# qway/nerfmeshes

Measured on AMD Instinct MI355X. Metric: rendered rays/sec (64+128 samples, 8x256 MLP), lego scene geometry, higher is better.
Workload: dtype f32; 1 GPU; nerf-synthetic lego: 8x256 coarse+fine MLP, 64 coarse + 128 fine samples, 800x800 view per step per rank, bounds [2,6], seeded weights/orbit poses; chunk_rays=65536, parallelism=single GPU

## Files before the change

### nerfmeshes_amd/csrc/mlp_device_r3.h

```cpp
#pragma once
#include "mlp_device.h"

namespace nm {

struct NextChunks {
    const char* s0; int b0;
    const char* s1; int b1;
};

template <int NT, int KS1, int KS2, int NW, int LDSBUF, int KCH>
__device__ __forceinline__ void gemm_stage3(f32x4 (&acc)[NT], const float (&b1)[KS1],
                                            const float (&b2)[(KS2 > 0 ? KS2 : 1)], const char* gw,
                                            const NextChunks nx, char* lds, int& slot, f32x4 (&carry)[2],
                                            int wave, int lane) {
    constexpr int KS = KS1 + KS2;
    constexpr int NCH = (KS + KCH - 1) / KCH;
    constexpr int NB = NT / 4;
    constexpr int STEP_BYTES = NT * 256;
    static_assert(NT % 4 == 0 && NB >= 1, "tile count");
    static_assert(NCH >= 2, "every stage must span at least two chunks (DMA runs two chunks ahead)");
    f32x4 ab[3];
    ab[0] = carry[0];
    ab[1] = carry[1];
#pragma unroll
    for (int c = 0; c < NCH; ++c) {
        const int steps = (KS - c * KCH) < KCH ? (KS - c * KCH) : KCH;
        const int nblk = steps * NB;
        const int slot1 = slot == 2 ? 0 : slot + 1;
        const int slot2 = slot1 == 2 ? 0 : slot1 + 1;
        const char* src;
        int bytes;
        if (c + 2 < NCH) {
            const int nsteps = (KS - (c + 2) * KCH) < KCH ? (KS - (c + 2) * KCH) : KCH;
            src = gw + (c + 2) * KCH * STEP_BYTES; bytes = nsteps * STEP_BYTES;
        } else if (c + 2 == NCH) { src = nx.s0; bytes = nx.b0; }
        else { src = nx.s1; bytes = nx.b1; }
        char* dst = lds + slot2 * LDSBUF;
        const char* buf = lds + slot * LDSBUF + lane * 16;
        const char* nbuf = lds + slot1 * LDSBUF + lane * 16;
#pragma unroll
        for (int j = 0; j < nblk; ++j) {
            if (j == 0 && wave < NW / 2) stream_to_lds<NW>(src, dst, bytes, wave, lane);
            if (j == nblk / 2 && wave >= NW / 2) stream_to_lds<NW>(src, dst, bytes, wave, lane);
            const int ks = j / NB, blk = j % NB;
            const int s = c * KCH + ks;
            const float b = s < KS1 ? b1[s < KS1 ? s : 0] : b2[s >= KS1 ? s - KS1 : 0];
            const char* from = (j + 2 < nblk) ? buf + (j + 2) * 1024 : nbuf + (j + 2 - nblk) * 1024;
            const int r0 = (c * KCH * NB + j) % 3;
            ab[(r0 + 2) % 3] = *reinterpret_cast<const f32x4*>(from);
            __builtin_amdgcn_sched_barrier(0);
#pragma unroll
            for (int q = 0; q < 4; ++q)
                acc[blk * 4 + q] = __builtin_amdgcn_mfma_f32_16x16x4f32(ab[r0][q], b, acc[blk * 4 + q], 0, 0, 0);
        }
        __syncthreads();
        slot = slot1;
    }
    constexpr int TOTAL = KS * NB;
    carry[0] = ab[TOTAL % 3];
    carry[1] = ab[(TOTAL + 1) % 3];
}

template <int H, int FX, int FD, int NW, int KCH, bool FLAT = false, bool SKIP = false>
__global__ __launch_bounds__(NW * 64, H <= 128 ? 4 : 2) void mlp_kernel3(const MlpArgs args, const int num_layers,
                                                          const int density_only) {
    using N = Net<H, FX, FD, KCH>;
    static_assert(!(FLAT && SKIP), "the use_viewdirs = 0 heads have no colour branch to skip");
    static_assert(N::EX > KCH && N::KH >= 2 * KCH, "stages must span two chunks");
    extern __shared__ __attribute__((aligned(16))) char lds[];
    float* lds_bias = reinterpret_cast<float*>(lds + 3 * N::LDSBUF);
    const int nbias = H * (1 + num_layers) + H / 2 + 4;
    float* lds_walpha = lds_bias + nbias;
    float* lds_wrgb = lds_walpha + H;
    int* lds_vote = reinterpret_cast<int*>(lds_wrgb + 3 * H / 2);
    uint32_t* lds_claim = reinterpret_cast<uint32_t*>(lds_vote + 1);
    if (SKIP && threadIdx.x == 0) *lds_vote = 0;
    for (int i = threadIdx.x; i < nbias; i += NW * 64) lds_bias[i] = args.bias[i];
    for (int i = threadIdx.x; i < H; i += NW * 64) lds_walpha[i] = args.walpha[i];
    for (int i = threadIdx.x; i < ((FLAT && density_only == 2) ? 3 * H : 3 * H / 2); i += NW * 64) lds_wrgb[i] = args.wrgb[i];
    const int lane = threadIdx.x & 63;
    const int wave = __builtin_amdgcn_readfirstlane(threadIdx.x >> 6);
    const int g = lane >> 4, col = lane & 15;
    const float* tail_bias = lds_bias + nbias - 4;

    const int64_t wg_iters = mlp_wg_iters(args, NW * 16);
    auto hidden_next = [](const char* p) {
        return NextChunks{p, KCH * N::STEP, p + KCH * N::STEP, (N::KH - KCH < KCH ? N::KH - KCH : KCH) * N::STEP};
    };
    auto enc_next = [](const char* p, bool on) {
        return NextChunks{p, on ? KCH * N::STEP : 0, p + KCH * N::STEP,
                          on ? (N::EX - KCH < KCH ? N::EX - KCH : KCH) * N::STEP : 0};
    };
    auto dir_next = [](const char* p) { return NextChunks{p, KCH * N::STEPD, p + KCH * N::STEPD, KCH * N::STEPD}; };

    int slot = 0;
    f32x4 carry[2];
    if ((int64_t)blockIdx.x < wg_iters) {
        const NextChunks first = enc_next(args.wstream, true);
        stream_to_lds<NW>(first.s0, lds, first.b0, wave, lane);
        stream_to_lds<NW>(first.s1, lds + N::LDSBUF, first.b1, wave, lane);
    }
    __syncthreads();
    carry[0] = *reinterpret_cast<const f32x4*>(lds + lane * 16);
    carry[1] = *reinterpret_cast<const f32x4*>(lds + lane * 16 + 1024);

    int64_t next_it = 0;
    int turn = 0;
    constexpr bool TERM = SKIP && H > 128;
    const bool term = TERM && args.att != nullptr;
    auto att_entry = [&](int64_t t, uint32_t& k) -> float* {
        k = (uint32_t)t / args.att_blocks;
        return args.att + ((size_t)(uint32_t)t * NW + wave);
    };
    bool dead = false;
    auto claim_tile = [&](float& pre) -> uint32_t {
        uint32_t c = 0;
        if (lane == 0) c = atomicAdd(args.tile_queue, 1u);
        c = (uint32_t)__builtin_amdgcn_readfirstlane((int)c);
        pre = 0.0f;
        if (term) {
            const int64_t nx = (int64_t)gridDim.x + c;
            if (nx < wg_iters && nx >= (int64_t)args.att_blocks && lane < NW)
                pre = __hip_atomic_load(args.att + ((size_t)((uint32_t)nx - args.att_blocks) * NW + lane), __ATOMIC_RELAXED,
                                        __HIP_MEMORY_SCOPE_AGENT);
        }
        return c;
    };
    auto claim_word = [&](uint32_t c, float pre) -> uint32_t {
        const bool all_dead = term && __ballot(lane < NW && !(pre < -160.0f)) == 0;
        return c | (all_dead ? 0x80000000u : 0u);
    };
    for (int64_t it = blockIdx.x; it < wg_iters; it = SKIP ? next_it : it + gridDim.x) {
        bool has_next = !SKIP && it + gridDim.x < wg_iters;
        int64_t sample = (it * NW + wave) * 16 + col;
        bool valid = sample < args.n;
        if (SKIP && args.ray_tiles) {
            const uint32_t depth_slots = (uint32_t)args.samples >> 4;
            const uint32_t div = term ? args.att_blocks : depth_slots;
            const uint32_t q = (uint32_t)it / div, r = (uint32_t)it - q * div;
            const uint32_t block = term ? r : q;
            const int64_t ray_first = ((int64_t)block * NW + wave) * args.samples;
            sample = ray_first + ((term ? q : r) << 4) + col;
            valid = ray_first < args.n;
        }
        if (TERM && dead) {
            if (valid && g == 0) {
                f32x4 o4 = {0.0f, 0.0f, 0.0f, 0.0f};
                *reinterpret_cast<f32x4*>(args.out + 4 * sample) = o4;
            }
            uint32_t k;
            float* const entry = att_entry(it, k);
            if (lane == 0) __hip_atomic_store(entry, -1e30f, __ATOMIC_RELAXED, __HIP_MEMORY_SCOPE_AGENT);
            if (args.dead_count && threadIdx.x == 0) atomicAdd(args.dead_count, 1u);
            if (wave == 0) {
                float pre;
                const uint32_t c = claim_tile(pre);
                const uint32_t word = claim_word(c, pre);
                if (lane == 0) lds_claim[turn] = word;
            }
            __syncthreads();
            const uint32_t word = (uint32_t)__builtin_amdgcn_readfirstlane((int)lds_claim[turn]);
            turn ^= 1;
            next_it = (int64_t)gridDim.x + (word & 0x7fffffffu);
            dead = (word >> 31) != 0;
            continue;
        }
        const int64_t sidx = valid ? sample : args.n - 1;
        const SamplePD smp = fetch_sample(args, sidx);
        const float p[3] = {smp.px, smp.py, smp.pz}, d[3] = {smp.dx, smp.dy, smp.dz};
        const float dummy[1] = {0.0f};
        float encx[N::EX];
        encode<FX, N::EX>(encx, p, args.bands_xyz, g);
        NextChunks wrap = enc_next(args.wstream, has_next);

        f32x4 acc[N::NT];
        float in[N::KH];
        const char* gw = args.wstream;
        load_bias<N::NT>(acc, lds_bias, g);
        gemm_stage3<N::NT, N::EX, 0, NW, N::LDSBUF, KCH>(acc, encx, dummy, gw, hidden_next(gw + N::EX * N::STEP), lds, slot, carry, wave, lane);
        gw += N::EX * N::STEP;
        acc_to_operand<N::NT, false>(acc, in);
        if constexpr (TERM) {
            if (wave == 0) {
                float pre;
                const uint32_t claimed = claim_tile(pre);
                const uint32_t word = claim_word(claimed, pre);
                if (lane == 0) lds_claim[turn] = word;
            }
        } else if (SKIP && threadIdx.x == 0) lds_claim[turn] = atomicAdd(args.tile_queue, 1u);

        float sigma = 0.0f;
        bool empty_tile = false;
        const int trunk_iters = density_only ? num_layers - 1 : num_layers;
#pragma unroll 1
        for (int i = 0; i < trunk_iters; ++i) {
            const bool is_feat = i == num_layers - 1;
            float t_here = 0.0f, t_after = 0.0f, att_before = 0.0f;
            float* entry = nullptr;
            bool last_of_ray = false;
            if (term && is_feat) {
                uint32_t k;
                entry = att_entry(it, k);
                last_of_ray = (k << 4) + col + 1 == (uint32_t)args.samples;
                if (valid) {
                    t_here = args.c[sample];
                    if (!last_of_ray) t_after = args.c[sample + 1];
                    if (lane == 0 && k > 0)
                        att_before = __hip_atomic_load(entry - (size_t)args.att_blocks * NW, __ATOMIC_RELAXED, __HIP_MEMORY_SCOPE_AGENT);
                }
            }
            if (is_feat) sigma = alpha_gemv<H>(in, lds_walpha, g) + tail_bias[0];
            if (term && is_feat) {
                const float dist = (last_of_ray ? 1e10f : t_after - t_here) * nm_norm3(d[0], d[1], d[2]);
                const float a = 1.0f - expf(-(fmaxf(sigma, 0.0f) * dist));
                float c = log2f(((1.0f - a) + 1e-10f) + 0x1p-23f) + 0x1p-8f;
#pragma unroll
                for (int m = 1; m < 16; m <<= 1) c += __shfl_xor(c, m);
                if (lane == 0)
                    __hip_atomic_store(entry, valid ? att_before + c : -1e30f, __ATOMIC_RELAXED, __HIP_MEMORY_SCOPE_AGENT);
            }
            if (SKIP && is_feat) {
                const int epoch = (int)it + 1;
                const bool dense = valid && !(sigma <= 0.0f);
                if (dense) *lds_vote = epoch;
                __syncthreads();
                empty_tile = __builtin_amdgcn_readfirstlane(*lds_vote) != epoch;
                const uint32_t word = (uint32_t)__builtin_amdgcn_readfirstlane((int)lds_claim[turn]);
                next_it = (int64_t)gridDim.x + (word & 0x7fffffffu);
                dead = (word >> 31) != 0;
                turn ^= 1;
                has_next = next_it < wg_iters;
                wrap = enc_next(args.wstream, has_next);
                if (empty_tile) break;
            }
            const bool skip = !is_feat && ((args.skip_mask >> i) & 1u);
            const bool last_density = density_only && i == num_layers - 2;
            load_bias<N::NT>(acc, lds_bias + H * (1 + i), g);
            {
                const char* after = gw + N::KH * N::STEP;
                NextChunks nx = hidden_next(after);
                if (skip) nx = enc_next(after, true);
                else if (is_feat) nx = dir_next(after);
                else if (last_density) nx = wrap;
                gemm_stage3<N::NT, N::KH, 0, NW, N::LDSBUF, KCH>(acc, in, dummy, gw, nx, lds, slot, carry, wave, lane);
                gw = after;
            }
            if (skip) {
                const char* after = gw + N::EX * N::STEP;
                const NextChunks nx = last_density ? wrap : hidden_next(after);
                gemm_stage3<N::NT, N::EX, 0, NW, N::LDSBUF, KCH>(acc, encx, dummy, gw, nx, lds, slot, carry, wave, lane);
                gw = after;
            }
            acc_to_operand<N::NT, true>(acc, in);
        }

        if (empty_tile) {
            if (valid && g == 0) {
                f32x4 o4 = {0.0f, 0.0f, 0.0f, sigma};
                *reinterpret_cast<f32x4*>(args.out + 4 * sample) = o4;
            }
            if (args.skip_count && threadIdx.x == 0) atomicAdd(args.skip_count, 1u);
            if (has_next) {
                const int slot1 = slot == 2 ? 0 : slot + 1;
                const int slot2 = slot1 == 2 ? 0 : slot1 + 1;
                stream_to_lds<NW>(wrap.s0, lds + slot1 * N::LDSBUF, wrap.b0, wave, lane);
                stream_to_lds<NW>(wrap.s1, lds + slot2 * N::LDSBUF, wrap.b1, wave, lane);
                __syncthreads();
                slot = slot1;
                carry[0] = *reinterpret_cast<const f32x4*>(lds + slot * N::LDSBUF + lane * 16);
                carry[1] = *reinterpret_cast<const f32x4*>(lds + slot * N::LDSBUF + lane * 16 + 1024);
            }
            continue;
        }

        if (density_only) {
            sigma = alpha_gemv<H>(in, lds_walpha, g) + tail_bias[0];
            if (FLAT && density_only == 2) flat_head<H>(args, in, lds_wrgb, tail_bias, sigma, sample, valid, g);
            else if (valid && g == 0) args.out[sample] = sigma;
            continue;
        }

        f32x4 accd[N::NTD];
        float v[N::KD];
        load_bias<N::NTD>(accd, lds_bias + H * (1 + num_layers), g);
        float encd[N::ED];
        encode<FD, N::ED>(encd, d, args.bands_dir, g);
        gemm_stage3<N::NTD, N::KH, N::ED, NW, N::LDSBUF, KCH>(accd, in, encd, gw, wrap, lds, slot, carry, wave, lane);
        acc_to_operand<N::NTD, true>(accd, v);

        float rgb[3];
#pragma unroll
        for (int ch = 0; ch < 3; ++ch) {
            float part = 0.0f;
            const float* wr = lds_wrgb + (ch * 4 + g) * N::KD;
#pragma unroll
            for (int s = 0; s < N::KD; s += 4) {
                const f32x4 w4 = *reinterpret_cast<const f32x4*>(wr + s);
#pragma unroll
                for (int q = 0; q < 4; ++q) part = fmaf(v[s + q], w4[q], part);
            }
            const float x = group_sum(part) + tail_bias[1 + ch];
            rgb[ch] = 1.0f / (1.0f + expf(-x));
        }
        if (valid && g == 0) {
            f32x4 o4 = {rgb[0], rgb[1], rgb[2], sigma};
            *reinterpret_cast<f32x4*>(args.out + 4 * sample) = o4;
        }
    }
}

}
```

### nerfmeshes_amd/csrc/nerf_mlp.hip

```cpp
#include <cstdlib>
#include <iterator>
#include <vector>

#include "nm_internal.h"
#include "mlp_device.h"
#include "mlp_device_r3.h"
#include "mlp_device_b3.h"
#include "mlp_device_g.h"

namespace nm {

template <int H, int FX, int FD, int NW, int KCH>
static MlpPlan make_plan() {
    return MlpPlan{H, FX, FD, NW, KCH, 0, 2 * Net<H, FX, FD, KCH>::LDSBUF, &mlp_kernel<H, FX, FD, NW, KCH, false>,
                   NW * 16, 8 / NW, &mlp_kernel<H, FX, FD, NW, KCH, false, true>, 0, nullptr, nullptr};
}

template <int H, int FX, int FD, int NW, int KCH, bool SKIP = true>
static MlpPlan make_plan3() {
    return MlpPlan{H, FX, FD, NW, KCH, 0, 3 * Net<H, FX, FD, KCH>::LDSBUF, &mlp_kernel3<H, FX, FD, NW, KCH>,
                   NW * 16, 8 / NW, &mlp_kernel3<H, FX, FD, NW, KCH, true>, 0, nullptr, nullptr,
                   SKIP ? &mlp_kernel3<H, FX, FD, NW, KCH, false, SKIP> : nullptr};
}

static const MlpPlan g_tuned_plans[] = {
    make_plan3<256, 10, 4, 8, 8>(),
    make_plan3<128, 10, 4, 8, 8>(),
    make_plan<64, 10, 4, 8, 8>(),
    make_plan3<256, 6, 4, 8, 8>(),
    make_plan3<128, 6, 4, 8, 8, false>(),
    make_plan<64, 6, 4, 8, 8>(),
};

void generic_plans_a(std::vector<MlpPlan>&);
void generic_plans_b(std::vector<MlpPlan>&);
void generic_plans_c(std::vector<MlpPlan>&);
void generic_plans_d(std::vector<MlpPlan>&);
void generic_plans_s(std::vector<MlpPlan>&);
void generic_plans_a_long(std::vector<MlpPlan>&);
void generic_plans_b_long(std::vector<MlpPlan>&);
void generic_plans_c_long(std::vector<MlpPlan>&);
void generic_plans_d_long(std::vector<MlpPlan>&);
void generic_plans_s_long(std::vector<MlpPlan>&);
void generic_plans_s_long_upper(std::vector<MlpPlan>&);

static const std::vector<MlpPlan>& all_plans() {
    static const std::vector<MlpPlan> plans = [] {
        std::vector<MlpPlan> v(std::begin(g_tuned_plans), std::end(g_tuned_plans));
        generic_plans_a(v); generic_plans_b(v); generic_plans_c(v); generic_plans_d(v); generic_plans_s(v);
        generic_plans_a_long(v); generic_plans_b_long(v); generic_plans_c_long(v); generic_plans_d_long(v); generic_plans_s_long(v); generic_plans_s_long_upper(v);
        return v;
    }();
    return plans;
}

struct B3Plan {
    int H, FX, FD;
    void (*kernel)(const MlpArgs, const int, const int);
    int chunk_units;
};
static const B3Plan g_b3_plans[] = {
    {256, 10, 4, &mlp_kernel_b3<256, 10, 4, 8>, B3_CHUNK_UNITS},
    {256, 6, 4, &mlp_kernel_b3<256, 6, 4, 8>, B3_CHUNK_UNITS},
    {128, 10, 4, &mlp_kernel_b3<128, 10, 4, 8, 8>, 8},
    {128, 6, 4, &mlp_kernel_b3<128, 6, 4, 8, 8>, 8},
    {64, 10, 4, &mlp_kernel_b3<64, 10, 4, 8, 3>, 3},
    {64, 6, 4, &mlp_kernel_b3<64, 6, 4, 8, 3>, 3},
};
static const B3Plan* find_b3_plan(int H, int FX, int FD) {
    for (const B3Plan& p : g_b3_plans)
        if (p.H == H && p.FX == FX && p.FD == FD) return &p;
    return nullptr;
}
bool has_b3_kernel(int H, int FX, int FD) { return find_b3_plan(H, FX, FD) != nullptr; }

const MlpPlan* find_mlp_plan(int H, int FX, int FD) {
    for (const MlpPlan& p : all_plans())
        if (!p.generic_nt && p.H == H && p.FX == FX && p.FD == FD) return &p;
    return nullptr;
}

const MlpPlan* find_generic_plan(int H, int L, bool long_encoding) {
    const int want = long_encoding ? G_LONG_VARIANT : 0;
    for (const MlpPlan& p : all_plans())
        if (p.generic_nt && p.variant == want && p.H >= H && forward_lds_bytes(p, H, L, 0) <= 160 * 1024) return &p;
    return nullptr;
}

int mlp_plan_info(const MlpPlan* p, int* nw) {
    *nw = p->NW;
    return p->generic_nt ? 1000 + p->generic_nt : p->variant;
}

int forward_lds_bytes(const MlpPlan& p, int H, int L, int head_floats) {
    if (p.generic_nt)
        return g_lds_bytes(p.ring_bytes, p.generic_nt, L, p.variant == G_LONG_VARIANT ? G_ENC_PARTS : 1);
    return p.ring_bytes + tuned_cache_bytes(H, L, head_floats);
}

static bool ray_termination_enabled() {
    const char* e = std::getenv("NM_RAY_TERMINATION");
    return !(e && e[0] == '0' && e[1] == 0);
}

int launch_mlp(const nm_mlp* m, const MlpArgs& args_in, int density_only, hipStream_t stream) {
    const MlpPlan* p = m->plan;
    if (args_in.n <= 0) return 0;
    MlpArgs args = args_in;
    if (!(args.skip_empty && p->kernel_skip && density_only == 0 && m->precision == NM_PREC_F32)) args.skip_empty = 0;
    args.ray_tiles = args.skip_empty && (args.mode == MODE_RAYS || args.mode == MODE_VIEW) && args.samples % 16 == 0;
    if (args.ray_tiles && mlp_wg_iters(args, p->wg_samples) > INT32_MAX) args.ray_tiles = 0;
    if (args.skip_empty && (!m->d_tile_queue || mlp_wg_iters(args, p->wg_samples) > INT32_MAX)) args.skip_empty = args.ray_tiles = 0;
    args.tile_queue = nullptr;
    if (!args.skip_empty) args.skip_count = nullptr;
    float* const att = args.ray_tiles ? args.att : nullptr;
    args.att = nullptr;
    args.att_blocks = 0;
    DeviceGuard guard(m->device);
    const int L = m->desc.num_layers, H = m->desc.hidden_size;
    NM_REQUIRE(density_only != 2 || (m->precision == NM_PREC_F32 && p->kernel_flat), "no kernel for use_viewdirs=0 networks in this plan");
    auto kernel = density_only == 2 ? p->kernel_flat : (args.skip_empty ? p->kernel_skip : p->kernel);
    if (m->precision == NM_PREC_BF16X3) {
        const B3Plan* b = find_b3_plan(H, m->desc.num_encoding_fn_xyz, m->desc.num_encoding_fn_dir);
        NM_REQUIRE(b && m->d_stream_b3, "no bf16x3 kernel for this network");
        const int lds_bytes = 3 * b->chunk_units * B3_UNIT + tuned_cache_bytes(H, L, 3 * H / 2 + 32);
        NM_REQUIRE(lds_bytes <= 160 * 1024, "LDS budget exceeded (bf16x3 ring + bias cache): too many layers");
        if (int rc = ensure_dynamic_lds((const void*)b->kernel, lds_bytes)) return rc;
        MlpArgs a = args;
        a.wstream = static_cast<const char*>(m->d_stream_b3);
        const unsigned grid = persistent_grid((a.n + 127) / 128, m->num_cus);
        hipLaunchKernelGGL(b->kernel, dim3(grid), dim3(512), lds_bytes, stream, a, L, density_only);
        NM_HIP_CHECK(hipGetLastError());
        return 0;
    }
    const int lds_bytes = forward_lds_bytes(*p, H, L, density_only == 2 ? 3 * H : 3 * H / 2);
    NM_REQUIRE(lds_bytes <= 160 * 1024, "LDS budget exceeded (ring + bias cache)");
    if (int rc = ensure_dynamic_lds((const void*)kernel, lds_bytes)) return rc;
    const int64_t wg_iters = mlp_wg_iters(args, p->wg_samples);
    unsigned grid = persistent_grid(wg_iters, (int64_t)m->num_cus * p->wg_per_cu);
    if (args.skip_empty) {
        const int64_t resident = (int64_t)m->num_cus * p->wg_per_cu * (p->H <= 128 ? 2 : 1);
        grid = (unsigned)(wg_iters < resident ? wg_iters : resident);
        args.tile_queue = m->d_tile_queue + (size_t)(__atomic_fetch_add(&m->tile_queue_turn, 1u, __ATOMIC_RELAXED) % TILE_QUEUE_SLOTS) * TILE_QUEUE_STRIDE;
        NM_HIP_CHECK(hipMemsetAsync(args.tile_queue, 0, sizeof(uint32_t), stream));
        const int64_t depth_slots = args.samples / 16, ray_blocks = att ? wg_iters / depth_slots : 0;
        const int64_t table = depth_slots * ray_blocks * p->NW;
        if (att && p->H > 128 && ray_blocks >= 2 * (int64_t)grid && table <= args.att_floats && ray_termination_enabled()) {
            args.att = att;
            args.att_blocks = (uint32_t)ray_blocks;
            NM_HIP_CHECK(hipMemsetAsync(att, 0, (size_t)table * sizeof(float), stream));
        }
    }
    if (!args.att) args.dead_count = nullptr;
    hipLaunchKernelGGL(kernel, dim3(grid), dim3(p->NW * 64), lds_bytes, stream, args, (int)m->desc.num_layers, density_only);
    NM_HIP_CHECK(hipGetLastError());
    return 0;
}

}
```

### nerfmeshes_amd/csrc/nm_internal.h

```cpp
#pragma once
#include <hip/hip_runtime.h>
#include <stdint.h>
#include <stdio.h>
#include <string.h>
#include <string>

#include "../../include/nerfmeshes_hip.h"
#include "mlp_pack.h"

namespace nm {

void set_error(const std::string& msg);

#define NM_HIP_CHECK(expr)                                                                   \
    do {                                                                                     \
        hipError_t _e = (expr);                                                              \
        if (_e != hipSuccess) {                                                              \
            ::nm::set_error(std::string(#expr) + ": " + hipGetErrorString(_e));              \
            return 1;                                                                        \
        }                                                                                    \
    } while (0)

#define NM_REQUIRE(cond, msg)                                                                \
    do {                                                                                     \
        if (!(cond)) {                                                                       \
            ::nm::set_error(std::string(msg) + " [" #cond "]");                              \
            return 2;                                                                        \
        }                                                                                    \
    } while (0)

constexpr int KC = 8;
constexpr int MAX_FREQ_XYZ = 32;
constexpr int MAX_FREQ_DIR = 32;

enum MlpMode : int { MODE_POINTS = 0, MODE_RAYS = 1, MODE_GRID = 2, MODE_VIEW = 3 };

struct RayGen {
    float rot[9];
    float origin[3];
    int32_t height, width;
    float focal;
    int32_t enabled;
    int32_t ndc;
    float ndc_near, c_w, c_h, two_near, m_two_near;
    int64_t first;
};

__device__ __forceinline__ float nm_norm3(float x, float y, float z) {
    return sqrtf(fmaf(z, z, fmaf(y, y, x * x)));
}

__device__ __forceinline__ void nm_ndc_ray(float near32, float c_w, float c_h, float two_near, float m_two_near,
                                           float (&o)[3], float (&d)[3]) {
    const float t = -(near32 + o[2]) / d[2];
    float q[3];
#pragma unroll
    for (int a = 0; a < 3; ++a) { const float td = t * d[a]; q[a] = o[a] + td; }
    const float o0 = (c_w * q[0]) / q[2];
    const float o1 = (c_h * q[1]) / q[2];
    const float rq = 1.0f / q[2];
    const float o2 = 1.0f + rq * two_near;
    const float d0 = c_w * (d[0] / d[2] - q[0] / q[2]);
    const float d1 = c_h * (d[1] / d[2] - q[1] / q[2]);
    const float d2 = rq * m_two_near;
    o[0] = o0; o[1] = o1; o[2] = o2;
    d[0] = d0; d[1] = d1; d[2] = d2;
}

__device__ __forceinline__ void nm_gen_ray(const RayGen& g, int64_t ray, float (&o)[3], float (&d)[3]) {
    const int64_t pix = g.first + ray;
    const int row = (int)(pix / g.width), colx = (int)(pix - (int64_t)row * g.width);
    const float x = ((float)colx - (float)(g.width * 0.5)) / g.focal;
    const float y = -((float)row - (float)(g.height * 0.5)) / g.focal;
    const float z = -1.0f;
    const float n = nm_norm3(x, y, z);
    const float dx = x / n, dy = y / n, dz = z / n;
#pragma unroll
    for (int a = 0; a < 3; ++a) {
        d[a] = (dx * g.rot[3 * a] + dy * g.rot[3 * a + 1]) + dz * g.rot[3 * a + 2];
        o[a] = g.origin[a];
    }
    if (g.ndc) nm_ndc_ray(g.ndc_near, g.c_w, g.c_h, g.two_near, g.m_two_near, o, d);
}

struct MlpArgs {
    const char* wstream;
    const float* bias;
    const float* walpha;
    const float* wrgb;
    float bands_xyz[MAX_FREQ_XYZ];
    float bands_dir[MAX_FREQ_DIR];
    uint32_t skip_mask;
    int32_t mode;
    const float* a;
    const float* b;
    const float* c;
    int64_t n;
    int64_t first;
    int32_t samples;
    int32_t origins_per_ray;
    int32_t n1, n2;
    float* out;
    float* tape_h;
    float* tape_feat;
    float* tape_v;
    uint64_t* mask_h;
    uint64_t* mask_v;
    int64_t tiles;
    float* tape_encx;
    float* tape_encd;
    int32_t tape_v_ld;
    int32_t tape_skip_h0;
    RayGen gen;
    const void* g_tab;
    int32_t g_nsx, g_idx, g_chx;
    int32_t g_nsd, g_idd, g_chd;
    int32_t g_h, g_hd;
    int32_t skip_empty;
    int32_t ray_tiles;
    uint32_t* skip_count;
    uint32_t* tile_queue;
    float* att;
    int64_t att_floats;
    uint32_t att_blocks;
    uint32_t* dead_count;
};

__host__ __device__ inline int64_t mlp_wg_iters(const MlpArgs& a, int wg_samples) {
    if (a.ray_tiles) {
        const int rays_per_tile = wg_samples / 16;
        return (a.n / a.samples + rays_per_tile - 1) / rays_per_tile * (a.samples / 16);
    }
    return (a.n + wg_samples - 1) / wg_samples;
}

struct MlpBwdArgs {
    const char* wstream;
    const float* walpha;
    const float* wrgb;
    const float* radiance;
    const float* grad_out;
    const uint64_t* mask_h;
    const uint64_t* mask_v;
    int64_t n, tiles;
    float* d_h;
    float* d_feat;
    float* d_v;
    float* d_last;
    const float* tape_h;
    const float* tape_feat;
    const float* tape_v;
    int32_t g_h, g_hd;
    int32_t stop_at_xyz0;
};

struct WeightPtrs { const float* p[T_COUNT]; };

struct MlpPlan {
    int H, FX, FD, NW, KCH, variant;
    int ring_bytes;
    void (*kernel)(const MlpArgs, const int, const int);
    int wg_samples;
    int wg_per_cu;
    void (*kernel_flat)(const MlpArgs, const int, const int);
    int generic_nt;
    void (*kernel_tape)(const MlpArgs, const int, const int);
    void (*kernel_bwd)(const MlpBwdArgs, const int, const int);
    void (*kernel_skip)(const MlpArgs, const int, const int);
};

int ensure_dynamic_lds(const void* kernel, int bytes);

struct DeviceGuard {
    int prev = -1;
    explicit DeviceGuard(int want) {
        int cur = -1;
        if (hipGetDevice(&cur) == hipSuccess && cur != want && hipSetDevice(want) == hipSuccess) prev = cur;
    }
    ~DeviceGuard() { if (prev >= 0) (void)hipSetDevice(prev); }
};

constexpr int TILE_QUEUE_SLOTS = 16, TILE_QUEUE_STRIDE = 32;

inline unsigned persistent_grid(int64_t wg_iters, int64_t resident) {
    int64_t grid = wg_iters < resident * 4 ? wg_iters : resident * 4;
    if (wg_iters > grid) {
        const int64_t rounds = (wg_iters + grid - 1) / grid;
        grid = (wg_iters + rounds - 1) / rounds;
    }
    return (unsigned)grid;
}

inline int tuned_cache_bytes(int H, int L, int head_floats) { return ((H * (1 + L) + H / 2 + 4 + H + head_floats) * 4 + 255) & ~255; }

int forward_lds_bytes(const MlpPlan& p, int H, int L, int head_floats);

MlpArgs ray_mode_args(const nm_mlp* m, const float* d_origins, int origins_per_ray, const float* d_dirs, const float* d_t, int64_t rays,
                      int32_t samples, float* d_radiance);

struct DwgGemmGeometry { int wa, wb, ta, tb, nba, nbb, out_pad; int64_t in_pad; };
DwgGemmGeometry dwg_gemm_geometry(int out, int64_t in);
struct DwgEpilogue { float* out; const float* bias; const float* mask; int64_t ld; int act; };
int dwg_gemm(const float* A, int out, int lda, const float* B, int64_t in, int64_t ldb, int rows, float* partial, hipStream_t stream,
             const DwgEpilogue* epilogue = nullptr);

constexpr int DW_MAX_JOBS = 16;
constexpr int HEAD_MAX_PARTS = 512;
struct DwReduceJob { const float* partial; const float* partial_bias; float* out; float* out_bias; int32_t out_ld, out_col0; };
struct DwReduceBatch { DwReduceJob job[DW_MAX_JOBS]; };
void launch_head_reduce(const float* partial, const float* partial_bias, int parts, int elems, float* out, float* out_bias,
                        hipStream_t stream);

int nm_mlp_eval_render_internal(nm_mlp* m, const RayGen* gen, const float* d_origins, int origins_per_ray, const float* d_dirs,
                                const float* d_t, int64_t rays, int32_t samples, float* d_radiance, float* d_att, int64_t att_floats,
                                hipStream_t stream);

}

struct nm_mlp {
    nm_mlp_desc desc;
    int device;
    const nm::MlpPlan* plan;
    void* d_blob;
    size_t blob_bytes;
    nm::MlpArgs base;
    nm::MlpBwdArgs bwd;
    int32_t* d_index;
    size_t blob_floats;
    int64_t flops_full, flops_density;
    int num_cus;
    int precision;
    void* d_stream_b3;
    float* d_tmp_b3;
    int32_t* d_index_b3;
    size_t b3_units;
    void* d_enc_tab;
    void* lw;
    unsigned long long* d_check;
    int64_t refresh_count;
    size_t plain_off;
    uint32_t* d_tile_queue;
    mutable uint32_t tile_queue_turn;
};
```

Baseline: 656,200 rays/s.

## Prefetch and encode next claimed tile's samples into LDS during trunk layers

In the early-termination persistent kernel, waves now fetch the next claimed tile's sample positions, directions and t values in the middle of the current tile's trunk layers. They positionally encode them and park the results in an extra LDS area. The next iteration reads the encoding and t values from LDS instead of global memory, hiding fetch and encode latency behind the GEMM work. The cost is extra LDS per workgroup, which could reduce occupancy, plus more register pressure and added complexity.

```diff
diff --git a/nerfmeshes_amd/csrc/mlp_device_r3.h b/nerfmeshes_amd/csrc/mlp_device_r3.h
--- a/nerfmeshes_amd/csrc/mlp_device_r3.h
+++ b/nerfmeshes_amd/csrc/mlp_device_r3.h
@@ -113,6 +113,17 @@
         return args.att + ((size_t)(uint32_t)t * NW + wave);
     };
     bool dead = false;
+    const bool park = TERM && term && args.park != 0;
+    constexpr int PARK_VEC = NW * 64;
+    typedef float f32x2 __attribute__((ext_vector_type(2)));
+    auto park_slot = [&]() -> f32x4* {
+        return reinterpret_cast<f32x4*>(lds + 3 * N::LDSBUF + tuned_cache_bytes(H, num_layers, 3 * H / 2) + wave * 1024 + lane * 16);
+    };
+    auto park_t = [&](int which) -> f32x2* {
+        return reinterpret_cast<f32x2*>(lds + 3 * N::LDSBUF + tuned_cache_bytes(H, num_layers, 3 * H / 2) + 5 * PARK_VEC * 16 + which * PARK_VEC * 8 +
+                                        wave * 512 + lane * 8);
+    };
+    bool parked = false;
     auto claim_tile = [&](float& pre) -> uint32_t {
         uint32_t c = 0;
         if (lane == 0) c = atomicAdd(args.tile_queue, 1u);
@@ -145,7 +156,9 @@
         }
         if (TERM && dead) {
             if (valid && g == 0) {
-                f32x4 o4 = {0.0f, 0.0f, 0.0f, 0.0f};
+                float zero;
+                asm volatile("v_mov_b32 %0, 0" : "=v"(zero));
+                f32x4 o4 = {zero, zero, zero, zero};
                 *reinterpret_cast<f32x4*>(args.out + 4 * sample) = o4;
             }
             uint32_t k;
@@ -165,12 +178,46 @@
             dead = (word >> 31) != 0;
             continue;
         }
-        const int64_t sidx = valid ? sample : args.n - 1;
-        const SamplePD smp = fetch_sample(args, sidx);
-        const float p[3] = {smp.px, smp.py, smp.pz}, d[3] = {smp.dx, smp.dy, smp.dz};
         const float dummy[1] = {0.0f};
-        float encx[N::EX];
-        encode<FX, N::EX>(encx, p, args.bands_xyz, g);
+        float encx[N::EX], d[3];
+        bool from_park = false;
+        if constexpr (TERM) {
+            from_park = parked;
+            parked = false;
+        }
+#if NM_PARK_RAW
+        float pr[3];
+        if (TERM && from_park) {
+            const f32x4 raw = park_slot()[0];
+            const f32x4 dir = park_slot()[4 * PARK_VEC];
+            d[0] = dir[0]; d[1] = dir[1]; d[2] = dir[2];
+            pr[0] = raw[0]; pr[1] = raw[1]; pr[2] = raw[2];
+        } else {
+            const int64_t sidx = valid ? sample : args.n - 1;
+            const SamplePD smp = fetch_sample(args, sidx);
+            pr[0] = smp.px; pr[1] = smp.py; pr[2] = smp.pz;
+            d[0] = smp.dx; d[1] = smp.dy; d[2] = smp.dz;
+        }
+        encode<FX, N::EX>(encx, pr, args.bands_xyz, g);
+        if (false)
+#endif
+        if (TERM && from_park) {
+#pragma unroll
+            for (int v = 0; v < (N::EX + 3) / 4; ++v) {
+                const f32x4 e = park_slot()[v * PARK_VEC];
+#pragma unroll
+                for (int q = 0; q < 4; ++q)
+                    if (4 * v + q < N::EX) encx[4 * v + q] = e[q];
+            }
+            const f32x4 dir = park_slot()[4 * PARK_VEC];
+            d[0] = dir[0]; d[1] = dir[1]; d[2] = dir[2];
+        } else {
+            const int64_t sidx = valid ? sample : args.n - 1;
+            const SamplePD smp = fetch_sample(args, sidx);
+            const float p[3] = {smp.px, smp.py, smp.pz};
+            d[0] = smp.dx; d[1] = smp.dy; d[2] = smp.dz;
+            encode<FX, N::EX>(encx, p, args.bands_xyz, g);
+        }
         NextChunks wrap = enc_next(args.wstream, has_next);
 
         f32x4 acc[N::NT];
@@ -195,6 +242,45 @@
 #pragma unroll 1
         for (int i = 0; i < trunk_iters; ++i) {
             const bool is_feat = i == num_layers - 1;
+            if constexpr (TERM) {
+                if (park && i == (wave < NW / 2 ? 1 : 2)) {
+                    const uint32_t word = (uint32_t)__builtin_amdgcn_readfirstlane((int)lds_claim[turn]);
+                    const int64_t nit = (int64_t)gridDim.x + (word & 0x7fffffffu);
+                    if (nit < wg_iters && (word >> 31) == 0) {
+                        const uint32_t q = (uint32_t)nit / args.att_blocks, r = (uint32_t)nit - q * args.att_blocks;
+                        const int64_t ray_first = ((int64_t)r * NW + wave) * args.samples;
+                        const int64_t nsample = ray_first + (q << 4) + col;
+                        const bool nvalid = ray_first < args.n;
+                        const SamplePD smp = fetch_sample(args, nvalid ? nsample : args.n - 1);
+                        f32x2 tt = {0.0f, 0.0f};
+                        if (nvalid) {
+                            tt[0] = args.c[nsample];
+                            if ((q << 4) + col + 1 != (uint32_t)args.samples) tt[1] = args.c[nsample + 1];
+                        }
+#if NM_PARK_RAW
+                        const f32x4 raw = {smp.px, smp.py, smp.pz, 0.0f};
+                        park_slot()[0] = raw;
+                        float e[N::EX] = {};
+                        if (false)
+#else
+                        const float p[3] = {smp.px, smp.py, smp.pz};
+                        float e[N::EX];
+                        encode<FX, N::EX>(e, p, args.bands_xyz, g);
+#endif
+#pragma unroll
+                        for (int v = 0; v < (N::EX + 3) / 4; ++v) {
+                            f32x4 e4;
+#pragma unroll
+                            for (int c4 = 0; c4 < 4; ++c4) e4[c4] = 4 * v + c4 < N::EX ? e[4 * v + c4 < N::EX ? 4 * v + c4 : 0] : 0.0f;
+                            park_slot()[v * PARK_VEC] = e4;
+                        }
+                        const f32x4 dir = {smp.dx, smp.dy, smp.dz, 0.0f};
+                        park_slot()[4 * PARK_VEC] = dir;
+                        *park_t(turn ^ 1) = tt;
+                        parked = true;
+                    }
+                }
+            }
             float t_here = 0.0f, t_after = 0.0f, att_before = 0.0f;
             float* entry = nullptr;
             bool last_of_ray = false;
@@ -203,8 +289,14 @@
                 entry = att_entry(it, k);
                 last_of_ray = (k << 4) + col + 1 == (uint32_t)args.samples;
                 if (valid) {
-                    t_here = args.c[sample];
-                    if (!last_of_ray) t_after = args.c[sample + 1];
+                    if (from_park) {
+                        const f32x2 tt = *park_t(turn);
+                        t_here = tt[0];
+                        t_after = tt[1];
+                    } else {
+                        t_here = args.c[sample];
+                        if (!last_of_ray) t_after = args.c[sample + 1];
+                    }
                     if (lane == 0 && k > 0)
                         att_before = __hip_atomic_load(entry - (size_t)args.att_blocks * NW, __ATOMIC_RELAXED, __HIP_MEMORY_SCOPE_AGENT);
                 }
diff --git a/nerfmeshes_amd/csrc/nerf_mlp.hip b/nerfmeshes_amd/csrc/nerf_mlp.hip
--- a/nerfmeshes_amd/csrc/nerf_mlp.hip
+++ b/nerfmeshes_amd/csrc/nerf_mlp.hip
@@ -116,6 +116,7 @@
     float* const att = args.ray_tiles ? args.att : nullptr;
     args.att = nullptr;
     args.att_blocks = 0;
+    args.park = 0;
     DeviceGuard guard(m->device);
     const int L = m->desc.num_layers, H = m->desc.hidden_size;
     NM_REQUIRE(density_only != 2 || (m->precision == NM_PREC_F32 && p->kernel_flat), "no kernel for use_viewdirs=0 networks in this plan");
@@ -133,9 +134,8 @@
         NM_HIP_CHECK(hipGetLastError());
         return 0;
     }
-    const int lds_bytes = forward_lds_bytes(*p, H, L, density_only == 2 ? 3 * H : 3 * H / 2);
+    int lds_bytes = forward_lds_bytes(*p, H, L, density_only == 2 ? 3 * H : 3 * H / 2);
     NM_REQUIRE(lds_bytes <= 160 * 1024, "LDS budget exceeded (ring + bias cache)");
-    if (int rc = ensure_dynamic_lds((const void*)kernel, lds_bytes)) return rc;
     const int64_t wg_iters = mlp_wg_iters(args, p->wg_samples);
     unsigned grid = persistent_grid(wg_iters, (int64_t)m->num_cus * p->wg_per_cu);
     if (args.skip_empty) {
@@ -149,8 +149,15 @@
             args.att = att;
             args.att_blocks = (uint32_t)ray_blocks;
             NM_HIP_CHECK(hipMemsetAsync(att, 0, (size_t)table * sizeof(float), stream));
+            const int park_bytes = TILE_PARK_BYTES * p->NW * 64;
+            if (L >= 3 && lds_bytes + park_bytes <= 160 * 1024) {
+                args.park = 1;
+                lds_bytes += park_bytes;
+            }
         }
     }
+    NM_REQUIRE(lds_bytes <= 160 * 1024, "LDS budget exceeded (ring + bias cache + park area)");
+    if (int rc = ensure_dynamic_lds((const void*)kernel, lds_bytes)) return rc;
     if (!args.att) args.dead_count = nullptr;
     hipLaunchKernelGGL(kernel, dim3(grid), dim3(p->NW * 64), lds_bytes, stream, args, (int)m->desc.num_layers, density_only);
     NM_HIP_CHECK(hipGetLastError());
diff --git a/nerfmeshes_amd/csrc/nm_internal.h b/nerfmeshes_amd/csrc/nm_internal.h
--- a/nerfmeshes_amd/csrc/nm_internal.h
+++ b/nerfmeshes_amd/csrc/nm_internal.h
@@ -123,6 +123,7 @@
     float* att;
     int64_t att_floats;
     uint32_t att_blocks;
+    uint32_t park;
     uint32_t* dead_count;
 };
 
@@ -191,7 +192,9 @@
     return (unsigned)grid;
 }
 
-inline int tuned_cache_bytes(int H, int L, int head_floats) { return ((H * (1 + L) + H / 2 + 4 + H + head_floats) * 4 + 255) & ~255; }
+__host__ __device__ inline int tuned_cache_bytes(int H, int L, int head_floats) { return ((H * (1 + L) + H / 2 + 4 + H + head_floats) * 4 + 255) & ~255; }
+
+constexpr int TILE_PARK_BYTES = 96;
 
 int forward_lds_bytes(const MlpPlan& p, int H, int L, int head_floats);
 
```

After: 648,300 rays/s. 0.988x the previous value.
